# ascentai/diy-gym

Hardware: AMD Instinct MI355X
Metric: env steps/sec (whole node) (higher is better)
Workload: dtype f32; 1 GPU; ur_high_5 x 16384 envs per GPU; envs_total=16384, substeps=2, auto_reset=True, launch=hipGraph replay of 8-step segments, parallelism=independent env shards x1, no collective, envs_per_wavefront=64, lds_bytes_per_workgroup=160512, parity=vs the C oracle only; parity with pybullet itself is UNPINNED (DESIGN.md 4)

## Files before the change

### diy_gym_amd/csrc/dg_kernels.h

```cpp
#pragma once
#include "dg_device.h"
#include "../../include/diygym_scene.h"
#include "../../include/diygym_hip.h"

namespace dg {

#define DG_MAX_LINKS 64
#define DG_MAX_BODIES 192

#define DG_CONSTANT __attribute__((address_space(4)))
typedef const int32_t DG_CONSTANT* cip;
typedef const float DG_CONSTANT* cfp;

struct DevScene {
  cip BI, LI, FI, SI, PI, GI, OI, IL;
  cfp BF, LF, FF, SF, PF, OF, FL, HF;
  cip PLB;
  int split_pgs;
  int early_dyn;
  int coll_split, cont2_off;
  int coll_wave;
  cfp GD;
  cip AM;
  cip SD;
// ... 70 lines not shown
    A.M.xx = L(o + 15); A.M.xy = L(o + 16); A.M.xz = L(o + 17); A.M.yy = L(o + 18); A.M.yz = L(o + 19); A.M.zz = L(o + 20);
    return A;
  }
  DGD void LAIset(int o, const AI& A) const {
    L(o) = A.I.xx; L(o + 1) = A.I.xy; L(o + 2) = A.I.xz; L(o + 3) = A.I.yy; L(o + 4) = A.I.yz; L(o + 5) = A.I.zz;
    _Pragma("unroll") for (int k = 0; k < 9; k++) L(o + 6 + k) = A.H.m[k];
    L(o + 15) = A.M.xx; L(o + 16) = A.M.xy; L(o + 17) = A.M.xz; L(o + 18) = A.M.yy; L(o + 19) = A.M.yz; L(o + 20) = A.M.zz;
  }
  DGD void LAIadd(int o, const AI& A) const {
    L(o) += A.I.xx; L(o + 1) += A.I.xy; L(o + 2) += A.I.xz; L(o + 3) += A.I.yy; L(o + 4) += A.I.yz; L(o + 5) += A.I.zz;
    _Pragma("unroll") for (int k = 0; k < 9; k++) L(o + 6 + k) += A.H.m[k];
    L(o + 15) += A.M.xx; L(o + 16) += A.M.xy; L(o + 17) += A.M.xz; L(o + 18) += A.M.yy; L(o + 19) += A.M.yz; L(o + 20) += A.M.zz;
  }

  DGD cip bi(int b) const { return sc.BI + b * DG_BI_STRIDE; }
  DGD cfp bf(int b) const { return sc.BF + b * DG_BF_STRIDE; }
  DGD cip li(int l) const { return sc.LI + l * DG_LI_STRIDE; }
  DGD cfp lf(int l) const { return sc.LF + l * DG_LF_STRIDE; }
  DGD cip plb(int b) const { return sc.PLB + b * PLB_STRIDE; }
  DGD cip pll(int l) const { return sc.PLL + l * PLL_STRIDE; }
  DGD bool fixed(int b) const { return bi(b)[DG_BI_FLAGS] & DG_BODY_FIXED; }
  DGD bool frozen(int b) const { return bi(b)[DG_BI_FLAGS] & DG_BODY_FROZEN; }
  DGD int ext_off(int b) const { return bi(b)[DG_BI_STATE_OFF] + (fixed(b) ? DG_BS_FIXED_END : DG_BS_FLOAT_END); }
  DGD float mass_scale(int gl) const { const int o = li(gl)[DG_LI_MASS_SCALE]; return o >= 0 ? S(o) : 1.0f; }
  DGD float ang_damping(int b) const { const int o = bi(b)[DG_BI_DYN_OFF]; return o >= 0 ? S(o) : sc.HF[DG_HF_ANG_DAMPING]; }
  DGD void link_inertia(int gl, float& m, V3& c, Sym3& Ic) const {
    cfp f = lf(gl); m = f[DG_LF_MASS]; c = v3(f[DG_LF_COM], f[DG_LF_COM + 1], f[DG_LF_COM + 2]); Ic = sym6(f + DG_LF_INERTIA);
    if (li(gl)[DG_LI_MASS_SCALE] >= 0) { const float s = mass_scale(gl); m *= s; Ic.xx *= s; Ic.xy *= s; Ic.xz *= s; Ic.yy *= s; Ic.yz *= s; Ic.zz *= s; }
  }

  DGD V3 base_pos(int b) const {
    if (frozen(b)) { cfp f = bf(b) + DG_BF_INIT_POS; return v3(f[0], f[1], f[2]); }
    int o = bi(b)[DG_BI_STATE_OFF]; return v3(S(o), S(o + 1), S(o + 2));
  }
  DGD Q4 base_quat(int b) const {
    if (frozen(b)) { cfp f = bf(b) + DG_BF_INIT_QUAT; Q4 q = {f[0], f[1], f[2], f[3]}; return q; }
    int o = bi(b)[DG_BI_STATE_OFF] + DG_BS_QUAT; Q4 q = {S(o), S(o + 1), S(o + 2), S(o + 3)}; return q;
  }

  DGD void link_world(int b, int gl, M3& R, V3& p) const {
    if (gl < 0) { R = frozen(b) ? qmat(base_quat(b)) : LR(plb(b)[PLB_R0]); p = base_pos(b); }
    else { int o = pll(gl)[PLL_POSE]; R = LR(o); p = L3(o + 6); }
  }

  DGD void joint_xform(int gl, float q, M3& Rpc, V3& r) const {
    cfp f = lf(gl);
    M3 RT; _Pragma("unroll") for (int k = 0; k < 9; k++) RT.m[k] = f[DG_LF_ROT + k];
    V3 pT = v3(f[DG_LF_POS], f[DG_LF_POS + 1], f[DG_LF_POS + 2]);
    V3 ax = v3(f[DG_LF_AXIS], f[DG_LF_AXIS + 1], f[DG_LF_AXIS + 2]);
    if (li(gl)[DG_LI_TYPE] == 0) { Rpc = mul(RT, rot_axis(ax, q)); r = pT; }
    else { Rpc = RT; r = pT + mul(RT, ax * q); }
  }

  DGD void kinematics_chain(int b) const {
    constexpr int N = 6;
    cip B = bi(b); const int first = B[DG_BI_FIRST_LINK], n = B[DG_BI_N_LINKS];
    M3 R = qmat(base_quat(b)); V3 p = base_pos(b);
    LRset(plb(b)[PLB_R0], R);
    float qv[N];
#pragma unroll
    for (int j = 0; j < N; j++) qv[j] = S(li(first + min(j, n - 1))[DG_LI_STATE_OFF] + DG_LS_Q);
#pragma unroll
    for (int j = 0; j < N; j++) {
      if (j < n) {
        const int gl = first + j; M3 Rpc; V3 r; joint_xform(gl, qv[j], Rpc, r);
        const M3 Rn = mul(R, Rpc); p = p + mul(R, r);
        const int o = pll(gl)[PLL_POSE];
        LRset(o, Rn); L3set(o + 6, p);
        const V3 c0 = v3(Rn.m[0], Rn.m[3], Rn.m[6]), c1 = v3(Rn.m[1], Rn.m[4], Rn.m[7]), c2 = cross(c0, c1);
        const M3 Rb = {{c0.x, c1.x, c2.x, c0.y, c1.y, c2.y, c0.z, c1.z, c2.z}}; R = Rb;
      }
    }
  }
  DGD void kinematics(int b, int qoff = -1) const {
    cip B = bi(b);
    if (B[DG_BI_FLAGS] & DG_BODY_FROZEN) return;
    if (qoff < 0 && plb(b)[PLB_CHAIN]) { kinematics_chain(b); return; }
    int first = B[DG_BI_FIRST_LINK], n = B[DG_BI_N_LINKS];
    M3 R0 = qmat(base_quat(b)); V3 p0 = base_pos(b);
    LRset(plb(b)[PLB_R0], R0);
    constexpr int KCH = 8;
    for (int i0 = 0; i0 < n; i0 += KCH) {
      float qv[KCH];
#pragma unroll
      for (int j = 0; j < KCH; j++) { const int i = min(i0 + j, n - 1); qv[j] = qoff >= 0 ? L(qoff + i) : S(li(first + i)[DG_LI_STATE_OFF] + DG_LS_Q); }
#pragma unroll
      for (int j = 0; j < KCH; j++) {
        const int i = i0 + j; if (i >= n) break;
        int gl = first + i, par = li(gl)[DG_LI_PARENT];
        M3 Rpc; V3 r; joint_xform(gl, qv[j], Rpc, r);
        M3 Rp; V3 pp;
        if (par < 0) { Rp = R0; pp = p0; } else { int o = pll(par)[PLL_POSE]; Rp = LR(o); pp = L3(o + 6); }
        int o = pll(gl)[PLL_POSE];
        LRset(o, mul(Rp, Rpc)); L3set(o + 6, pp + mul(Rp, r));
      }
    }
  }

  DGD void frame_state(int b, int fr, bool com, V3& p, Q4& q, V3& v, V3& w, bool want_vel) const {
    V3 off; Q4 qo; int gl;
    if (fr < 0) {
      gl = -1;
      if (com) { cfp f = bf(b); off = v3(f[DG_BF_REPORT_POS], f[DG_BF_REPORT_POS + 1], f[DG_BF_REPORT_POS + 2]);
        Q4 t = {f[DG_BF_REPORT_QUAT], f[DG_BF_REPORT_QUAT + 1], f[DG_BF_REPORT_QUAT + 2], f[DG_BF_REPORT_QUAT + 3]}; qo = t; }
      else { off = v3(0, 0, 0); Q4 t = {0, 0, 0, 1}; qo = t; }
    } else {
      gl = sc.FI[fr * DG_FI_STRIDE + DG_FI_LINK];
      cfp f = sc.FF + fr * DG_FF_STRIDE + (com ? DG_FF_COM_POS : DG_FF_POS);
      off = v3(f[0], f[1], f[2]); Q4 t = {f[3], f[4], f[5], f[6]}; qo = t;
    }
    M3 R; V3 o; link_world(b, gl, R, o);
    Q4 ql = gl < 0 ? base_quat(b) : qfrom_mat(R);
    p = o + mul(R, off); q = qnormalize(qmul(ql, qo));
    if (!want_vel) return;
    V3 wl = v3(0, 0, 0), vl = v3(0, 0, 0), po = base_pos(b);
    if (!fixed(b)) { int so = bi(b)[DG_BI_STATE_OFF]; vl = v3(S(so + DG_BS_LINVEL), S(so + DG_BS_LINVEL + 1), S(so + DG_BS_LINVEL + 2));
      wl = v3(S(so + DG_BS_ANGVEL), S(so + DG_BS_ANGVEL + 1), S(so + DG_BS_ANGVEL + 2)); }
    if (gl >= 0) {
      int first = bi(b)[DG_BI_FIRST_LINK];
      unsigned long long path = 0ull; for (int k = gl; k >= 0; k = li(k)[DG_LI_PARENT]) path |= 1ull << (k - first);
      for (int k = first; k <= gl; k++) {
        if (!((path >> (k - first)) & 1ull)) continue;
        int po_off = pll(k)[PLL_POSE]; M3 Rk = LR(po_off); V3 pk = L3(po_off + 6);
        cfp f = lf(k); V3 axw = mul(Rk, v3(f[DG_LF_AXIS], f[DG_LF_AXIS + 1], f[DG_LF_AXIS + 2]));
        float qd = S(li(k)[DG_LI_STATE_OFF] + DG_LS_QD);
        vl = vl + cross(wl, pk - po);
        if (li(k)[DG_LI_TYPE] == 0) wl = wl + axw * qd; else vl = vl + axw * qd;
        po = pk;
      }
    }
    w = wl; v = vl + cross(wl, p - po);
  }

// ... 402 lines not shown
```

### diy_gym_amd/csrc/dg_solver.h

```cpp
#pragma once
#include "dg_kernels.h"
#include "dg_hull.h"

namespace dg {

enum { PS_UPDATE = 0, PS_KIN, PS_COLLIDE, PS_ABA, PS_MINV, PS_ROWS, PS_PGS, PS_INTEGRATE, PS_OUTPUT, PS_PGS_MOTOR, PS_PGS_LIMIT, PS_PGS_CONTACT, PS_COUNT,
       PS_ROW = PS_COUNT + 12  };
template <bool PROF> struct Prof;
template <> struct Prof<false> { DGD void start() {} DGD void stamp(int) {} };
template <> struct Prof<true> {
  unsigned long long last, acc[PS_COUNT];
  DGD void start() { _Pragma("unroll") for (int k = 0; k < PS_COUNT; k++) acc[k] = 0ull; last = __builtin_amdgcn_s_memtime(); }
  DGD void stamp(int id) {
    unsigned long long t = __builtin_amdgcn_s_memtime();
    _Pragma("unroll") for (int k = 0; k < PS_COUNT; k++) if (k == id) acc[k] += t - last;
    last = t;
  }
};

struct WShape { int type, body, glink; M3 R; V3 p; float prm0, prm1, prm2, mu; int poff, npts; };

template <int LANES>
DGD void shape_world(const Lane<LANES>& ln, int sh, WShape& o) {
  cip si = ln.sc.SI + sh * DG_SI_STRIDE; cfp sf = ln.sc.SF + sh * DG_SF_STRIDE;
// ... 2291 lines not shown
    }
    float U[21];
#pragma unroll
    for (int k = 0; k < 21; k++) U[k] = 0.f;
    for (int k = 0; k < n; k++) {
      float col[6];
#pragma unroll
      for (int r = 0; r < 6; r++) col[r] = ln.L(jo + r * n + k);
#pragma unroll
      for (int r = 0; r < 6; r++)
#pragma unroll
        for (int c = 0; c <= r; c++) U[r * (r + 1) / 2 + c] += col[r] * col[c];
    }
#pragma unroll
    for (int r = 0; r < 6; r++) U[r * (r + 1) / 2 + r] += lam2;
    chol6(U);
    float y[6]; chol6_solve(U, dS, y);
    float Jv[6] = {0.f, 0.f, 0.f, 0.f, 0.f, 0.f};
    for (int k = 0; k < n; k++) {
      float t = 0.f;
#pragma unroll
      for (int r = 0; r < 6; r++) t += ln.L(jo + r * n + k) * y[r];
      float v0 = 0.f;
      if (nullsp) {
        float q = ln.L(qo + k), lo = rest[n + k], hi = rest[2 * n + k], rg = rest[3 * n + k];
        v0 = g0 * (rest[k] - q);
        if (q > hi) v0 += g1 * (hi - q) / rg;
        if (q < lo) v0 += g1 * (lo - q) / rg;
#pragma unroll
        for (int r = 0; r < 6; r++) Jv[r] += ln.L(jo + r * n + k) * v0;
      }
      ln.L(vo + k) = v0; ln.L(dto + k) = t;
    }
    float mx = 0.f;
    if (nullsp) {
      float z[6]; chol6_solve(U, Jv, z);
      for (int k = 0; k < n; k++) {
        float t = 0.f;
#pragma unroll
        for (int r = 0; r < 6; r++) t += ln.L(jo + r * n + k) * z[r];
        float d = ln.L(dto + k) + ln.L(vo + k) - t; ln.L(dto + k) = d; mx = fmaxf(mx, fabsf(d));
      }
    } else {
      for (int k = 0; k < n; k++) mx = fmaxf(mx, fabsf(ln.L(dto + k)));
    }
    const float scl = mx > maxang ? maxang / mx : 1.0f;
    for (int k = 0; k < n; k++) if (live) ln.L(qo + k) += scl * ln.L(dto + k);
  }
  return iters;
}

#define DG_IK_DEV_CHAIN 256
#define DG_IK_DEV_FULL 512
template <int LANES, int N, bool FULL = false, bool NS = false, bool ORN = false>
DGD int run_ik_chain(const Lane<LANES>& ln, int op, const float* act, bool live_lane, float* qout) {
  const DevScene& sc = ln.sc; cip oi = sc.OI + op * DG_OI_STRIDE;
  const int b = oi[DG_OI_BODY], fr = oi[DG_OI_FRAME], flags = oi[DG_OI_FLAGS];
  const bool use_orn = FULL ? ORN : (flags & DG_IK_USE_ORIENTATION) != 0, nullsp = FULL ? NS : (flags & DG_IK_NULLSPACE) != 0;
  const int first = ln.bi(b)[DG_BI_FIRST_LINK], n = FULL ? N : ln.bi(b)[DG_BI_N_LINKS];
  const int eel = FULL ? N - 1 : sc.FI[fr * DG_FI_STRIDE + DG_FI_LINK] - first;
  cfp rest = sc.FL + oi[DG_OI_FLIST]; cfp ff = sc.FF + fr * DG_FF_STRIDE;
  const V3 off = v3(ff[DG_FF_COM_POS], ff[DG_FF_COM_POS + 1], ff[DG_FF_COM_POS + 2]);
  const Q4 qoff = {ff[DG_FF_COM_QUAT], ff[DG_FF_COM_QUAT + 1], ff[DG_FF_COM_QUAT + 2], ff[DG_FF_COM_QUAT + 3]};
  const M3 R0 = ln.LR(ln.plb(b)[PLB_R0]); const V3 p0 = ln.base_pos(b);
  float q[N]; V3 ow[N], aw[N];
  float cR[N][9], cP[N][3]; bool rev[N];
  M3 Qprev = {{1.f, 0.f, 0.f, 0.f, 1.f, 0.f, 0.f, 0.f, 1.f}}, Qee = Qprev;
#pragma unroll
  for (int i = 0; i < N; i++) {
    q[i] = 0.f; rev[i] = true;
#pragma unroll
    for (int k = 0; k < 9; k++) cR[i][k] = 0.f;
#pragma unroll
    for (int k = 0; k < 3; k++) cP[i][k] = 0.f;
    if (FULL || i < n) {
      cfp f = ln.lf(first + i); q[i] = ln.S(ln.li(first + i)[DG_LI_STATE_OFF] + DG_LS_Q); rev[i] = FULL || ln.li(first + i)[DG_LI_TYPE] == 0;
      M3 RT; _Pragma("unroll") for (int k = 0; k < 9; k++) RT.m[k] = pin(f[DG_LF_ROT + k]);
      const V3 pT = v3(pin(f[DG_LF_POS]), pin(f[DG_LF_POS + 1]), pin(f[DG_LF_POS + 2]));
      const V3 ax = v3(pin(f[DG_LF_AXIS]), pin(f[DG_LF_AXIS + 1]), pin(f[DG_LF_AXIS + 2]));
      V3 u, v; tangent_basis(ax, u, v);
      const M3 Qi = {{u.x, v.x, ax.x, u.y, v.y, ax.y, u.z, v.z, ax.z}};
      const M3 RTp = mul(transpose(Qprev), mul(RT, Qi)); const V3 pTp = tmul(Qprev, pT);
#pragma unroll
      for (int k = 0; k < 9; k++) cR[i][k] = RTp.m[k];
      cP[i][0] = pTp.x; cP[i][1] = pTp.y; cP[i][2] = pTp.z;
      Qprev = Qi; if (FULL ? i == N - 1 : i == eel) Qee = Qi;
    }
  }
  const V3 offp = tmul(Qee, off);
  float nRest[N], nLo[N], nHi[N], nIrg[N];
#pragma unroll
  for (int i = 0; i < N; i++) {
    nRest[i] = 0.f; nLo[i] = -3.0e38f; nHi[i] = 3.0e38f; nIrg[i] = 0.f;
    if (nullsp && (FULL || i < n)) { nRest[i] = pin(rest[i]); nLo[i] = pin(rest[n + i]); nHi[i] = pin(rest[2 * n + i]); nIrg[i] = pin(frcp(rest[3 * n + i])); }
  }
  V3 pe; M3 Re;
  auto fk = [&]() {
    M3 R = R0; V3 p = p0; M3 Rl = R0; V3 pl = p0;
#pragma unroll
    for (int i = 0; i < N; i++) {
      if (FULL || i < n) {
        M3 RT; _Pragma("unroll") for (int k = 0; k < 9; k++) RT.m[k] = cR[i][k];
        p = p + mul(R, v3(cP[i][0], cP[i][1], cP[i][2]));
        const M3 C = mul(R, RT);
        const V3 c0 = v3(C.m[0], C.m[3], C.m[6]), c1 = v3(C.m[1], C.m[4], C.m[7]), c2 = v3(C.m[2], C.m[5], C.m[8]);
        if (FULL || rev[i]) {
          const float sn = __sinf(q[i]), cs = __cosf(q[i]);
          const V3 n0 = c0 * cs + c1 * sn, n1 = c1 * cs - c0 * sn;
          const M3 Rn = {{n0.x, n1.x, c2.x, n0.y, n1.y, c2.y, n0.z, n1.z, c2.z}}; R = Rn;
        } else { R = C; p = p + c2 * q[i]; }
        ow[i] = p; aw[i] = c2;
        if (FULL ? i == N - 1 : i == eel) { Rl = R; pl = p; }
      }
    }
    pe = pl + mul(Rl, offp); Re = Rl;
  };
  fk();
  const V3 tp = pe + v3(act[0], act[1], act[2]);
  M3 Tm = {{1.f, 0.f, 0.f, 0.f, 1.f, 0.f, 0.f, 0.f, 1.f}};
  if (use_orn) {
    const Q4 qe0 = qnormalize(qmul(qfrom_mat(mul(Re, transpose(Qee))), qoff));
    const Q4 tq = qmul(qe0, qfrom_euler(act[3], act[4], act[5]));
    Tm = mul(mul(qmat(tq), transpose(qmat(qoff))), Qee);
  }
  const float lam2 = nullsp ? sc.HF[DG_HF_IK_LAMBDA_SQ] : sc.HF[DG_HF_IK_JOINT_DAMPING], maxang = sc.HF[DG_HF_IK_MAX_ANGLE], g0 = sc.HF[DG_HF_IK_NULL_REST_GAIN], g1 = sc.HF[DG_HF_IK_NULL_LIMIT_GAIN];
  const float resid = sc.HF[DG_HF_IK_RESIDUAL];
  bool live = live_lane; int iters = 0;
  for (int it = 0; it < sc.ik_iters; it++) {
    if (it > 0) fk();
    const V3 ep = tp - pe;
    if (it > 0 && norm(ep) < resid) live = false;
    if (!__any(live)) break;
    iters += live ? 1 : 0;
    float dS[6] = {ep.x, ep.y, ep.z, 0.f, 0.f, 0.f};
    if (use_orn) {
      const float* T = Tm.m; const float* R = Re.m;
      const float tr = T[0] * R[0] + T[1] * R[1] + T[2] * R[2] + T[3] * R[3] + T[4] * R[4] + T[5] * R[5] + T[6] * R[6] + T[7] * R[7] + T[8] * R[8];
      const float m21 = T[3] * R[0] + T[4] * R[1] + T[5] * R[2], m12 = T[0] * R[3] + T[1] * R[4] + T[2] * R[5];
      const float m31 = T[6] * R[0] + T[7] * R[1] + T[8] * R[2], m13 = T[0] * R[6] + T[1] * R[7] + T[2] * R[8];
      const float m32 = T[6] * R[3] + T[7] * R[4] + T[8] * R[5], m23 = T[3] * R[6] + T[4] * R[7] + T[5] * R[8];
      const float sx = 0.5f * (m32 - m23), sy = 0.5f * (m13 - m31), sz = 0.5f * (m21 - m12);
      const float sn = fsqrt(sx * sx + sy * sy + sz * sz), an = atan2f(sn, 0.5f * (tr - 1.0f)), k = sn > 1e-12f ? fdiv(an, sn) : 1.0f;
      dS[3] = sx * k; dS[4] = sy * k; dS[5] = sz * k;
    }
    float U[21], Jv[6] = {0.f, 0.f, 0.f, 0.f, 0.f, 0.f}, v0[N], cols[N][6];
#pragma unroll
    for (int k = 0; k < 21; k++) U[k] = 0.f;
    auto column = [&](int i, float* col) {
      const V3 jl = (FULL || rev[i]) ? cross(aw[i], pe - ow[i]) : aw[i]; const V3 ja = ((FULL || rev[i]) && use_orn) ? aw[i] : v3(0.f, 0.f, 0.f);
      col[0] = jl.x; col[1] = jl.y; col[2] = jl.z; col[3] = ja.x; col[4] = ja.y; col[5] = ja.z;
    };
#pragma unroll
    for (int i = 0; i < N; i++) {
      v0[i] = 0.f;
      if (FULL || i < n) {
        if (nullsp) {
          v0[i] = g0 * (nRest[i] - q[i]);
          if (q[i] > nHi[i]) v0[i] += g1 * (nHi[i] - q[i]) * nIrg[i];
          if (q[i] < nLo[i]) v0[i] += g1 * (nLo[i] - q[i]) * nIrg[i];
        }
        if (FULL || i <= eel) {
          float* col = cols[i]; column(i, col);
#pragma unroll
          for (int r = 0; r < 6; r++) {
            Jv[r] += col[r] * v0[i];
#pragma unroll
            for (int c = 0; c <= r; c++) U[r * (r + 1) / 2 + c] += col[r] * col[c];
          }
        }
      }
    }
#pragma unroll
    for (int r = 0; r < 6; r++) U[r * (r + 1) / 2 + r] += lam2;
    chol6(U);
    float rhs[6], y[6];
#pragma unroll
    for (int r = 0; r < 6; r++) rhs[r] = dS[r] - Jv[r];
    chol6_solve(U, rhs, y);
    float dth[N], mx = 0.f;
#pragma unroll
    for (int i = 0; i < N; i++) {
      dth[i] = 0.f;
      if (FULL || i < n) {
        float t = 0.f;
        if (FULL || i <= eel) {
#pragma unroll
          for (int r = 0; r < 6; r++) t += cols[i][r] * y[r];
        }
        dth[i] = t + v0[i]; mx = fmaxf(mx, fabsf(dth[i]));
      }
    }
    const float scl = mx > maxang ? fdiv(maxang, mx) : 1.0f;
#pragma unroll
    for (int i = 0; i < N; i++) if ((FULL || i < n) && live) q[i] += scl * dth[i];
  }
#pragma unroll
  for (int i = 0; i < N; i++) qout[i] = q[i];
  return iters;
}

typedef float v2f __attribute__((ext_vector_type(2)));
DGD v2f sp2(float s) { v2f r = {s, s}; return r; }
DGD v2f fma2(v2f a, v2f b, v2f c) { return __builtin_elementwise_fma(a, b, c); }
struct P3 { v2f xy; float z; };
DGD P3 p3(V3 v) { P3 r; r.xy.x = v.x; r.xy.y = v.y; r.z = v.z; return r; }
DGD P3 colmul_acc(const P3& c0, const P3& c1, const P3& c2, float x, float y, float z, const P3& acc) {
  P3 r; r.xy = fma2(c2.xy, sp2(z), fma2(c1.xy, sp2(y), fma2(c0.xy, sp2(x), acc.xy))); r.z = fmaf(c2.z, z, fmaf(c1.z, y, fmaf(c0.z, x, acc.z))); return r;
}
DGD P3 colmul(const P3& c0, const P3& c1, const P3& c2, float x, float y, float z) {
  P3 r; r.xy = fma2(c2.xy, sp2(z), fma2(c1.xy, sp2(y), c0.xy * sp2(x))); r.z = fmaf(c2.z, z, fmaf(c1.z, y, c0.z * x)); return r;
}
template <int LANES, bool ORN>
DGD int run_ik_chain_pk(const Lane<LANES>& ln, int op, const float* act, bool live_lane, float* qout) {
  constexpr int N = 6;
  const DevScene& sc = ln.sc; cip oi = sc.OI + op * DG_OI_STRIDE;
  const int b = oi[DG_OI_BODY], fr = oi[DG_OI_FRAME];
  const int first = ln.bi(b)[DG_BI_FIRST_LINK];
  cfp rest = sc.FL + oi[DG_OI_FLIST]; cfp ff = sc.FF + fr * DG_FF_STRIDE;
  const V3 off = v3(ff[DG_FF_COM_POS], ff[DG_FF_COM_POS + 1], ff[DG_FF_COM_POS + 2]);
  const Q4 qoff = {ff[DG_FF_COM_QUAT], ff[DG_FF_COM_QUAT + 1], ff[DG_FF_COM_QUAT + 2], ff[DG_FF_COM_QUAT + 3]};
  const M3 R0 = ln.LR(ln.plb(b)[PLB_R0]); const V3 p0 = ln.base_pos(b);
  float q[N];
  float cR[N][9], cP[N][3];
  M3 Qprev = {{1.f, 0.f, 0.f, 0.f, 1.f, 0.f, 0.f, 0.f, 1.f}}, Qee = Qprev;
#pragma unroll
  for (int i = 0; i < N; i++) {
    cfp f = ln.lf(first + i); q[i] = ln.S(ln.li(first + i)[DG_LI_STATE_OFF] + DG_LS_Q);
    M3 RT; _Pragma("unroll") for (int k = 0; k < 9; k++) RT.m[k] = pin(f[DG_LF_ROT + k]);
    const V3 pT = v3(pin(f[DG_LF_POS]), pin(f[DG_LF_POS + 1]), pin(f[DG_LF_POS + 2]));
    const V3 ax = v3(pin(f[DG_LF_AXIS]), pin(f[DG_LF_AXIS + 1]), pin(f[DG_LF_AXIS + 2]));
    V3 u, v; tangent_basis(ax, u, v);
    const M3 Qi = {{u.x, v.x, ax.x, u.y, v.y, ax.y, u.z, v.z, ax.z}};
    const M3 RTp = mul(transpose(Qprev), mul(RT, Qi)); const V3 pTp = tmul(Qprev, pT);
#pragma unroll
    for (int k = 0; k < 9; k++) cR[i][k] = RTp.m[k];
    cP[i][0] = pTp.x; cP[i][1] = pTp.y; cP[i][2] = pTp.z;
    Qprev = Qi; if (i == N - 1) Qee = Qi;
  }
  const V3 offp = tmul(Qee, off);
  float nRest[N], nLo[N], nHi[N], nIrg[N];
#pragma unroll
  for (int i = 0; i < N; i++) { nRest[i] = pin(rest[i]); nLo[i] = pin(rest[N + i]); nHi[i] = pin(rest[2 * N + i]); nIrg[i] = pin(frcp(rest[3 * N + i])); }
  const P3 b0 = p3(v3(R0.m[0], R0.m[3], R0.m[6])), b1 = p3(v3(R0.m[1], R0.m[4], R0.m[7])), b2 = p3(v3(R0.m[2], R0.m[5], R0.m[8])), bp = p3(p0);
  P3 ow[N], aw[N], pe, e0, e1, e2;
  auto fk = [&]() {
    P3 c0 = b0, c1 = b1, c2 = b2, p = bp;
#pragma unroll
    for (int i = 0; i < N; i++) {
      const float* T = cR[i];
      p = colmul_acc(c0, c1, c2, cP[i][0], cP[i][1], cP[i][2], p);
      const P3 C0 = colmul(c0, c1, c2, T[0], T[3], T[6]), C1 = colmul(c0, c1, c2, T[1], T[4], T[7]), C2 = colmul(c0, c1, c2, T[2], T[5], T[8]);
      const float sn = __sinf(q[i]), cs = __cosf(q[i]);
      P3 n0, n1;
      n0.xy = fma2(C1.xy, sp2(sn), C0.xy * sp2(cs)); n0.z = fmaf(C1.z, sn, C0.z * cs);
      n1.xy = fma2(C0.xy, sp2(-sn), C1.xy * sp2(cs)); n1.z = fmaf(C0.z, -sn, C1.z * cs);
      c0 = n0; c1 = n1; c2 = C2; ow[i] = p; aw[i] = C2;
    }
    pe = colmul_acc(c0, c1, c2, offp.x, offp.y, offp.z, p); e0 = c0; e1 = c1; e2 = c2;
  };
  fk();
  const V3 pe0 = v3(pe.xy.x, pe.xy.y, pe.z);
  const V3 tp = pe0 + v3(act[0], act[1], act[2]);
  M3 Tm = {{1.f, 0.f, 0.f, 0.f, 1.f, 0.f, 0.f, 0.f, 1.f}};
  if (ORN) {
    const M3 Re = {{e0.xy.x, e1.xy.x, e2.xy.x, e0.xy.y, e1.xy.y, e2.xy.y, e0.z, e1.z, e2.z}};
    const Q4 qe0 = qnormalize(qmul(qfrom_mat(mul(Re, transpose(Qee))), qoff));
    const Q4 tq = qmul(qe0, qfrom_euler(act[3], act[4], act[5]));
    Tm = mul(mul(qmat(tq), transpose(qmat(qoff))), Qee);
  }
  const float lam2 = sc.HF[DG_HF_IK_LAMBDA_SQ], maxang = sc.HF[DG_HF_IK_MAX_ANGLE], g0 = sc.HF[DG_HF_IK_NULL_REST_GAIN], g1 = sc.HF[DG_HF_IK_NULL_LIMIT_GAIN];
  const float resid = sc.HF[DG_HF_IK_RESIDUAL];
  bool live = live_lane; int iters = 0;
  for (int it = 0; it < sc.ik_iters; it++) {
    if (it > 0) fk();
    const v2f epxy = v2f{tp.x, tp.y} - pe.xy; const float epz = tp.z - pe.z;
    if (it > 0 && fsqrt(epxy.x * epxy.x + epxy.y * epxy.y + epz * epz) < resid) live = false;
    if (!__any(live)) break;
    iters += live ? 1 : 0;
    v2f dA = epxy, dB = {0.f, 0.f}, dC = {epz, 0.f};
    if (ORN) {
      const P3 M0 = colmul(e0, e1, e2, Tm.m[0], Tm.m[1], Tm.m[2]), M1 = colmul(e0, e1, e2, Tm.m[3], Tm.m[4], Tm.m[5]), M2 = colmul(e0, e1, e2, Tm.m[6], Tm.m[7], Tm.m[8]);
      const float tr = M0.xy.x + M1.xy.y + M2.z;
      const float sx = 0.5f * (M2.xy.y - M1.z), sy = 0.5f * (M0.z - M2.xy.x), sz = 0.5f * (M1.xy.x - M0.xy.y);
      const float sn = fsqrt(sx * sx + sy * sy + sz * sz), an = atan2f(sn, 0.5f * (tr - 1.0f)), k = sn > 1e-12f ? fdiv(an, sn) : 1.0f;
      dB = v2f{sx * k, sy * k}; dC.y = sz * k;
    }
    float U00 = 0.f, U22 = 0.f, U44 = 0.f; v2f U1 = {0.f, 0.f}, U2a = U1, U3a = U1, U3b = U1, U4a = U1, U4b = U1, U5a = U1, U5b = U1, U5c = U1;
    v2f JvA = U1, JvB = U1, JvC = U1, cA[N], cB[N], cC[N]; float v0[N];
#pragma unroll
    for (int i = 0; i < N; i++) {
      float v = g0 * (nRest[i] - q[i]);
      if (q[i] > nHi[i]) v += g1 * (nHi[i] - q[i]) * nIrg[i];
      if (q[i] < nLo[i]) v += g1 * (nLo[i] - q[i]) * nIrg[i];
      v0[i] = v;
      const v2f dxy = pe.xy - ow[i].xy; const float dz = pe.z - ow[i].z; const P3& a = aw[i];
      const v2f pa = {a.xy.y, -a.xy.x}, pd = {dxy.y, -dxy.x};
      const v2f A = fma2(pa, sp2(dz), -(pd * sp2(a.z)));
      const float lz = a.xy.x * dxy.y - a.xy.y * dxy.x;
      const v2f B = a.xy, C = {lz, a.z};
      cA[i] = A; cB[i] = B; cC[i] = C;
      JvA = fma2(A, sp2(v), JvA); JvB = fma2(B, sp2(v), JvB); JvC = fma2(C, sp2(v), JvC);
      U00 = fmaf(A.x, A.x, U00); U1 = fma2(A, sp2(A.y), U1);
      U2a = fma2(A, sp2(B.x), U2a); U22 = fmaf(B.x, B.x, U22);
      U3a = fma2(A, sp2(B.y), U3a); U3b = fma2(B, sp2(B.y), U3b);
      U4a = fma2(A, sp2(C.x), U4a); U4b = fma2(B, sp2(C.x), U4b); U44 = fmaf(C.x, C.x, U44);
      U5a = fma2(A, sp2(C.y), U5a); U5b = fma2(B, sp2(C.y), U5b); U5c = fma2(C, sp2(C.y), U5c);
    }
    float U[21] = {U00 + lam2, U1.x, U1.y + lam2, U2a.x, U2a.y, U22 + lam2, U3a.x, U3a.y, U3b.x, U3b.y + lam2,
                   U4a.x, U4a.y, U4b.x, U4b.y, U44 + lam2, U5a.x, U5a.y, U5b.x, U5b.y, U5c.x, U5c.y + lam2};
    chol6(U);
    const float rhs[6] = {dA.x - JvA.x, dA.y - JvA.y, dB.x - JvB.x, dB.y - JvB.y, dC.x - JvC.x, dC.y - JvC.y};
    float y[6]; chol6_solve(U, rhs, y);
// ... 28 lines not shown
DGD M3 qmat_x(Q4 q) {
#pragma clang fp contract(off)
  const float n = q.x * q.x + q.y * q.y + q.z * q.z + q.w * q.w, s = n > 0.f ? 2.0f * __frcp_rn(n) : 0.f;
  const float xs = q.x * s, ys = q.y * s, zs = q.z * s;
  const float wx = q.w * xs, wy = q.w * ys, wz = q.w * zs, xx = q.x * xs, xy = q.x * ys, xz = q.x * zs, yy = q.y * ys, yz = q.y * zs, zz = q.z * zs;
  M3 R = {{1.f - (yy + zz), xy - wz, xz + wy, xy + wz, 1.f - (xx + zz), yz - wx, xz - wy, yz + wx, 1.f - (xx + yy)}};
  return R;
}
DGD float spool_up(float w, float a, float k) {
#pragma clang fp contract(off)
  const float d = a - w; const float p = d * k; return w + p;
}
DGD float mul_sep(float a, float b) {
#pragma clang fp contract(off)
  const float p = a * b; return p;
}
DGD V3 mulx(const M3& R, V3 v) {
#pragma clang fp contract(off)
  return v3(R.m[0] * v.x + R.m[1] * v.y + R.m[2] * v.z, R.m[3] * v.x + R.m[4] * v.y + R.m[5] * v.z, R.m[6] * v.x + R.m[7] * v.y + R.m[8] * v.z);
}
template <int LANES>
DGD void apply_frame_wrench(const Lane<LANES>& ln, int b, int fr, V3 f, V3 pos, V3 t, bool link_frame) {
#pragma clang fp contract(off)
  const DevScene& sc = ln.sc;
  const int gl = fr < 0 ? -1 : sc.FI[fr * DG_FI_STRIDE + DG_FI_LINK];
  V3 F = f, T = t, P = pos;
  if (link_frame) {
    V3 fp; M3 R;
    if (gl < 0) {
      const Q4 qb = ln.base_quat(b); const V3 pb = ln.base_pos(b);
      cfp ff = fr >= 0 ? sc.FF + fr * DG_FF_STRIDE + DG_FF_COM_POS : ln.bf(b) + DG_BF_REPORT_POS;
      const V3 off = v3(ff[0], ff[1], ff[2]); const Q4 qo = {ff[3], ff[4], ff[5], ff[6]};
      const V3 ro = mulx(qmat_x(qb), off); fp = v3(pb.x + ro.x, pb.y + ro.y, pb.z + ro.z); R = qmat_x(qnormalize_x(qmul_x(qb, qo)));
    } else { V3 fv, fw; Q4 fq; ln.frame_state(b, fr, true, fp, fq, fv, fw, false); R = qmat_x(fq); }
    F = mulx(R, f); T = mulx(R, t);
    const V3 rp = mulx(R, pos); P = v3(fp.x + rp.x, fp.y + rp.y, fp.z + rp.z);
  }
  if (!ln.fixed(b)) {
    const V3 bp = ln.base_pos(b), r = v3(P.x - bp.x, P.y - bp.y, P.z - bp.z);
    const V3 tq = v3((r.y * F.z - r.z * F.y) + T.x, (r.z * F.x - r.x * F.z) + T.y, (r.x * F.y - r.y * F.x) + T.z); const int eo = ln.ext_off(b);
    ln.Sset(eo, ln.S(eo) + F.x); ln.Sset(eo + 1, ln.S(eo + 1) + F.y); ln.Sset(eo + 2, ln.S(eo + 2) + F.z);
    ln.Sset(eo + 3, ln.S(eo + 3) + tq.x); ln.Sset(eo + 4, ln.S(eo + 4) + tq.y); ln.Sset(eo + 5, ln.S(eo + 5) + tq.z);
  }
  for (int k = gl; k >= 0; k = ln.li(k)[DG_LI_PARENT]) {
    const int po = ln.pll(k)[PLL_POSE], lo = ln.li(k)[DG_LI_STATE_OFF]; cfp lf = ln.lf(k);
    const M3 Rk = ln.LR(po); const V3 pk = ln.L3(po + 6), a = v3(lf[DG_LF_AXIS], lf[DG_LF_AXIS + 1], lf[DG_LF_AXIS + 2]);
    const V3 axw = v3(Rk.m[0] * a.x + Rk.m[1] * a.y + Rk.m[2] * a.z, Rk.m[3] * a.x + Rk.m[4] * a.y + Rk.m[5] * a.z, Rk.m[6] * a.x + Rk.m[7] * a.y + Rk.m[8] * a.z);
    const V3 r = v3(P.x - pk.x, P.y - pk.y, P.z - pk.z), m = v3((r.y * F.z - r.z * F.y) + T.x, (r.z * F.x - r.x * F.z) + T.y, (r.x * F.y - r.y * F.x) + T.z);
    const float tau = ln.li(k)[DG_LI_TYPE] == 0 ? axw.x * m.x + axw.y * m.y + axw.z * m.z : axw.x * F.x + axw.y * F.y + axw.z * F.z;
    ln.Sset(lo + DG_LS_TORQUE, ln.S(lo + DG_LS_TORQUE) + tau);
  }
}

template <int LANES>
DGD void run_update_ops(const Lane<LANES>& ln, const float* act_row, uint64_t mask, int only_body = -1, int skip_body = -1, int32_t* diag = nullptr) {
  const DevScene& sc = ln.sc; int ik_ord = -1;
  for (int op = 0; op < sc.nops; op++) {
    cip oi = sc.OI + op * DG_OI_STRIDE; cfp of = sc.OF + op * DG_OF_STRIDE; const int code = oi[DG_OI_CODE];
    if (code == DG_OP_IK_CONTROL) ik_ord++;
    if (code < DG_OP_JOINT_CONTROL || code > DG_OP_ADMITTANCE) continue;
    if ((only_body >= 0 && oi[DG_OI_BODY] != only_body) || oi[DG_OI_BODY] == skip_body) continue;
    if (!((mask >> oi[DG_OI_SLOT]) & 1ull)) continue;
    const float* a = act_row + oi[DG_OI_IO_OFF]; cip il = sc.IL + oi[DG_OI_ILIST]; const int n = oi[DG_OI_N];
    if (code == DG_OP_JOINT_CONTROL) {
      const int mode = oi[DG_OI_FLAGS];
      for (int k = 0; k < n; k++) {
        const int lo = ln.li(il[k])[DG_LI_STATE_OFF];
        if (mode == DG_JC_POSITION) { ln.Sset(lo + DG_LS_TARGET_POS, a[k]); ln.Sset(lo + DG_LS_TARGET_VEL, 0.f); }
        else if (mode == DG_JC_VELOCITY) { ln.Sset(lo + DG_LS_TARGET_VEL, a[k]); ln.Sset(lo + DG_LS_TARGET_POS, 0.f); }
        else ln.Sset(lo + DG_LS_TORQUE, a[k]);
      }
    } else if (code == DG_OP_IK_CONTROL) {
      const int b = oi[DG_OI_BODY];
      float av[6] = {a[0], a[1], a[2], 0.f, 0.f, 0.f};
      if (oi[DG_OI_FLAGS] & DG_IK_USE_ORIENTATION) { av[3] = a[3]; av[4] = a[4]; av[5] = a[5]; }
      if (oi[DG_OI_FLAGS] & DG_IK_DEV_CHAIN) {
        float qs[6]; int ik_it;
        const int fl = oi[DG_OI_FLAGS];
        if ((fl & DG_IK_DEV_FULL) && (fl & DG_IK_NULLSPACE) && (fl & DG_IK_USE_ORIENTATION)) ik_it = run_ik_chain_pk<LANES, true>(ln, op, av, ln.valid, qs);
        else if ((fl & DG_IK_DEV_FULL) && (fl & DG_IK_NULLSPACE)) ik_it = run_ik_chain_pk<LANES, false>(ln, op, av, ln.valid, qs);
        else ik_it = run_ik_chain<LANES, 6>(ln, op, av, ln.valid, qs);
        if (diag && ln.valid && ik_ord < DG_DIAG_N_IK) diag[(size_t)DG_DIAG_STRIDE * ln.env + DG_DIAG_IK_ITERS + ik_ord] = ik_it;
        const int first = ln.bi(b)[DG_BI_FIRST_LINK];
        for (int k = 0; k < n; k++) {
          const int lo = ln.li(il[k])[DG_LI_STATE_OFF], j = il[k] - first; float v = qs[0];
#pragma unroll
          for (int c = 1; c < 6; c++) v = (j == c) ? qs[c] : v;
          ln.Sset(lo + DG_LS_TARGET_POS, v); ln.Sset(lo + DG_LS_TARGET_VEL, 0.f);
        }
        continue;
      }
      { const int ik_it = run_ik(ln, op, av, ln.valid);
        if (diag && ln.valid && ik_ord < DG_DIAG_N_IK) diag[(size_t)DG_DIAG_STRIDE * ln.env + DG_DIAG_IK_ITERS + ik_ord] = ik_it; }
      for (int k = 0; k < n; k++) {
        const int lo = ln.li(il[k])[DG_LI_STATE_OFF];
        ln.Sset(lo + DG_LS_TARGET_POS, ln.L(sc.tr_off + (il[k] - ln.bi(b)[DG_BI_FIRST_LINK]))); ln.Sset(lo + DG_LS_TARGET_VEL, 0.f);
      }
      ln.kinematics(b);
    } else if (code == DG_OP_ADMITTANCE) {
      const int b = oi[DG_OI_BODY], first = ln.bi(b)[DG_BI_FIRST_LINK], nl = ln.bi(b)[DG_BI_N_LINKS];
      V3 fp, fv, fw; Q4 fq; ln.frame_state(b, oi[DG_OI_FRAME], true, fp, fq, fv, fw, false);
      const V3 pw = fp + mul(qmat(fq), v3(of[0], of[1], of[2]));
      const int eel = sc.FI[oi[DG_OI_FRAME] * DG_FI_STRIDE + DG_FI_LINK];
      const V3 F = v3(a[0], a[1], a[2]), T = v3(a[3], a[4], a[5]), g = v3(sc.gx, sc.gy, sc.gz); cfp tgt = sc.FL + oi[DG_OI_FLIST];
      for (int k = 0; k < n; k++) {
        const int gl = il[k], lo = ln.li(gl)[DG_LI_STATE_OFF], po = ln.pll(gl)[PLL_POSE]; cfp f = ln.lf(gl);
        const M3 Rj = ln.LR(po); const V3 oj = ln.L3(po + 6), axw = mul(Rj, v3(f[DG_LF_AXIS], f[DG_LF_AXIS + 1], f[DG_LF_AXIS + 2]));
        const bool rev = ln.li(gl)[DG_LI_TYPE] == 0;
        bool anc = false; for (int i = eel; i >= 0; i = ln.li(i)[DG_LI_PARENT]) if (i == gl) anc = true;
        float tau = 0.f;
        if (anc) tau += rev ? dot(F, cross(axw, pw - oj)) + dot(T, axw) : dot(F, axw);
        for (int i = first; i < first + nl; i++) {
          bool sub = false; for (int q = i; q >= 0; q = ln.li(q)[DG_LI_PARENT]) if (q == gl) sub = true;
          if (!sub) continue;
          cfp fi2 = ln.lf(i); const int pi2 = ln.pll(i)[PLL_POSE];
          const V3 cw = ln.L3(pi2 + 6) + mul(ln.LR(pi2), v3(fi2[DG_LF_COM], fi2[DG_LF_COM + 1], fi2[DG_LF_COM + 2])); const V3 w8 = g * (fi2[DG_LF_MASS] * ln.mass_scale(i));
          tau -= rev ? dot(w8, cross(axw, cw - oj)) : dot(w8, axw);
        }
        tau += of[3] * (tgt[k] - ln.S(lo + DG_LS_Q)) - of[4] * ln.S(lo + DG_LS_QD);
        ln.Sset(lo + DG_LS_TORQUE, ln.S(lo + DG_LS_TORQUE) + tau);
      }
    } else if (code == DG_OP_EXTERNAL_FORCE) {
      const int b = oi[DG_OI_BODY]; if (ln.fixed(b)) continue;
      apply_frame_wrench(ln, b, -1, v3(a[0], a[1], a[2]), v3(of[0], of[1], of[2]), v3(0.f, 0.f, 0.f), false);
    } else if (code == DG_OP_PROPELLOR) {
      const int b = oi[DG_OI_BODY], so = sc.addon_off + oi[DG_OI_STATE_OFF];
      const float w = spool_up(ln.S(so), a[0], of[2]); ln.Sset(so, w);
      if (ln.fixed(b)) continue;
      apply_frame_wrench(ln, b, oi[DG_OI_FRAME], v3(0.f, 0.f, mul_sep(of[0], w)), v3(0.f, 0.f, 0.f), v3(0.f, 0.f, mul_sep(of[1], w)), true);
    }
  }
}

template <int LANES>
// ... 234 lines not shown
```

### diy_gym_amd/csrc/dg_step_par_body.inc

```
  constexpr int reset_mode = DG_PAR_RESET;
  extern __shared__ float smem[];
  const int wave = threadIdx.x >> 6, lane = threadIdx.x & 63;
  const int env = blockIdx.x * 64 + lane; const bool exists = env < sc.num_envs; const int e = exists ? env : sc.num_envs - 1;
  const bool doit = exists && (!reset_mode || reset_mask == nullptr || reset_mask[e] != 0);
  if (reset_mode && !__any(doit)) return;
  const bool valid = reset_mode ? doit : exists;
  const float* act_row = actions ? actions + (size_t)e * sc.act_dim : nullptr;
  const unsigned long long t_start = PROF ? __builtin_amdgcn_s_memtime() : 0ull; (void)t_start;
  if (wave == 3) {
    Lane<64> ln(sc, mt, smem + lane, state + e, e, valid);
    if (reset_mode) __syncthreads();
    DG_WAVE_STAMP(0); __syncthreads();
    if (sc.early_dyn) {
      early_dynamics(ln, 1);
      if (sc.coll_split) collide<64, 64>(ln, sc.npairs / 2, 0x7fffffff, sc.cont2_off);
    }
    DG_WAVE_STAMP(1); __syncthreads();
    for (int k = 0; k < sc.substeps; k++) {
      __syncthreads();
      if (sc.coll_split && !(sc.early_dyn && k == 0)) collide<64, 64>(ln, sc.npairs / 2, 0x7fffffff, sc.cont2_off);
      __syncthreads();
      if (!substep_contact_free(ln) && split_decide_follow(ln, 0u, false)) __syncthreads();
      __syncthreads();
    }
    DG_WAVE_STAMP(2); __syncthreads();
    run_output_ops(ln, nullptr, (valid && rew) ? rew + (size_t)e * sc.rew_dim : nullptr, (valid && term) ? term + (size_t)e * sc.term_dim : nullptr,
                   (valid && rew_sum) ? rew_sum + e : nullptr, (valid && term_flag) ? term_flag + e : nullptr, OUT_REW_TERM);
    DG_WAVE_STAMP(3);
    return;
  }
  if (wave == 2) {
    Lane<64> ln(sc, mt, smem + lane, state + e, e, valid);
    if (reset_mode) __syncthreads();
    DG_WAVE_STAMP(0); __syncthreads();
    if (sc.early_dyn) {
      collide<64, 64>(ln, 0, sc.coll_split ? sc.npairs / 2 : 0x7fffffff);
      early_dynamics(ln, 0);
    }
    DG_WAVE_STAMP(1); __syncthreads();
    for (int k = 0; k < sc.substeps; k++) {
      __syncthreads();
      if (sc.coll_wave && !(sc.early_dyn && k == 0)) collide<64, 64>(ln, 0, sc.coll_split ? sc.npairs / 2 : 0x7fffffff);
      __syncthreads();
      if (!substep_contact_free(ln) && split_decide_follow(ln, false, false)) __syncthreads();
      __syncthreads();
    }
    DG_WAVE_STAMP(2); __syncthreads();
    run_output_ops(ln, (valid && obs) ? obs + (size_t)e * sc.obs_dim : nullptr, nullptr, nullptr, nullptr, nullptr, OUT_OBS_REST);
    DG_WAVE_STAMP(3);
    return;
  }
  if (wave == 1) {
    Lane<64> ln(sc, mt, smem + lane, state + e, e, valid);
    if (reset_mode) __syncthreads();
    ln.kinematics(sc.helper_body);
    DG_WAVE_STAMP(0); __syncthreads();
    if (act_row) run_update_ops(ln, act_row, mask, sc.helper_body, -1, diag);
    DG_WAVE_STAMP(1); __syncthreads();
    for (int k = 0; k < sc.substeps; k++) helper_substep(ln, sc.early_dyn && k == 0, k == sc.substeps - 1);
    ln.kinematics(sc.helper_body);
    DG_WAVE_STAMP(2); __syncthreads();
    run_output_ops(ln, (valid && obs) ? obs + (size_t)e * sc.obs_dim : nullptr, nullptr, nullptr, nullptr, nullptr, OUT_JOINT_OF, sc.helper_body);
    DG_WAVE_STAMP(3);
    return;
  }
  Lane<64> ln(sc, mt, smem + lane, state + e, e, valid);
  Prof<PROF> prof; prof.start();
  if (reset_mode) { if (doit) { ln.Sset(DG_ST_STEP, 0.0f); run_reset_ops(ln); } __syncthreads(); }
  for (int b = 0; b < sc.nba; b++) if (b != sc.helper_body) ln.kinematics(b);
  __syncthreads();
  prof.stamp(PS_KIN);
  if (act_row) run_update_ops(ln, act_row, mask, -1, sc.helper_body, diag);
  if (!reset_mode) ln.Sset(DG_ST_STEP, ln.S(DG_ST_STEP) + 1.0f);
  __syncthreads();
  prof.stamp(PS_UPDATE);
  sim_step<64, PROF, true>(ln, diag, prof);
  for (int b = 0; b < sc.nba; b++) if (b != sc.helper_body) ln.kinematics(b);
  __syncthreads();
  prof.stamp(PS_KIN);
  run_output_ops(ln, (valid && obs) ? obs + (size_t)e * sc.obs_dim : nullptr, nullptr, nullptr, nullptr, nullptr, OUT_JOINT_NOT_OF, sc.helper_body);
  prof.stamp(PS_OUTPUT);
  if constexpr (PROF) { if (lane == 0) for (int k = 0; k < PS_COUNT; k++) cycles[(size_t)blockIdx.x * PS_ROW + k] = prof.acc[k]; }
```

Before: 182.3 million env-steps/s.

## Hand off pre-step link kinematics to idle waves and overlap with IK start

When early dynamics and split collision are enabled, the full link-pose kinematics for the helper body and first regular body moves to waves 3 and 2, which are otherwise idle before the first barrier. The IK-owning waves only write the base rotation to LDS and then begin IK. A Handover functor places the first barrier inside the IK routine, just before its forward-kinematics pass, so per-op constant loads and setup overlap with the pose computation on other waves. This shortens the serial kinematics-then-update critical path, at the cost of extra template plumbing and barrier placement that depends on IK being reached.

Measured after the change: 188.8 million env-steps/s (median of 6 runs). 3.6% higher.

```diff
diff --git a/diy_gym_amd/csrc/dg_kernels.h b/diy_gym_amd/csrc/dg_kernels.h
--- a/diy_gym_amd/csrc/dg_kernels.h
+++ b/diy_gym_amd/csrc/dg_kernels.h
@@ -146,11 +146,12 @@
     else { Rpc = RT; r = pT + mul(RT, ax * q); }
   }
 
-  DGD void kinematics_chain(int b) const {
+  DGD void base_rot_to_lds(int b) const { if (!frozen(b)) LRset(plb(b)[PLB_R0], qmat(base_quat(b))); }
+  DGD void kinematics_chain(int b, bool base_rot = true) const {
     constexpr int N = 6;
     cip B = bi(b); const int first = B[DG_BI_FIRST_LINK], n = B[DG_BI_N_LINKS];
     M3 R = qmat(base_quat(b)); V3 p = base_pos(b);
-    LRset(plb(b)[PLB_R0], R);
+    if (base_rot) LRset(plb(b)[PLB_R0], R);
     float qv[N];
 #pragma unroll
     for (int j = 0; j < N; j++) qv[j] = S(li(first + min(j, n - 1))[DG_LI_STATE_OFF] + DG_LS_Q);
@@ -166,13 +167,13 @@
       }
     }
   }
-  DGD void kinematics(int b, int qoff = -1) const {
+  DGD void kinematics(int b, int qoff = -1, bool base_rot = true) const {
     cip B = bi(b);
     if (B[DG_BI_FLAGS] & DG_BODY_FROZEN) return;
-    if (qoff < 0 && plb(b)[PLB_CHAIN]) { kinematics_chain(b); return; }
+    if (qoff < 0 && plb(b)[PLB_CHAIN]) { kinematics_chain(b, base_rot); return; }
     int first = B[DG_BI_FIRST_LINK], n = B[DG_BI_N_LINKS];
     M3 R0 = qmat(base_quat(b)); V3 p0 = base_pos(b);
-    LRset(plb(b)[PLB_R0], R0);
+    if (base_rot) LRset(plb(b)[PLB_R0], R0);
     constexpr int KCH = 8;
     for (int i0 = 0; i0 < n; i0 += KCH) {
       float qv[KCH];
diff --git a/diy_gym_amd/csrc/dg_solver.h b/diy_gym_amd/csrc/dg_solver.h
--- a/diy_gym_amd/csrc/dg_solver.h
+++ b/diy_gym_amd/csrc/dg_solver.h
@@ -2367,8 +2367,15 @@
 
 #define DG_IK_DEV_CHAIN 256
 #define DG_IK_DEV_FULL 512
-template <int LANES, int N, bool FULL = false, bool NS = false, bool ORN = false>
-DGD int run_ik_chain(const Lane<LANES>& ln, int op, const float* act, bool live_lane, float* qout) {
+struct NoHandover { DGD void operator()() const {} };
+template <class F>
+struct Handover {
+  F f; bool done;
+  DGD Handover(F fn, bool d) : f(fn), done(d) {}
+  DGD void operator()() { if (!done) { done = true; f(); } }
+};
+template <int LANES, int N, bool FULL = false, bool NS = false, bool ORN = false, class HO = NoHandover>
+DGD int run_ik_chain(const Lane<LANES>& ln, int op, const float* act, bool live_lane, float* qout, HO&& ho = HO()) {
   const DevScene& sc = ln.sc; cip oi = sc.OI + op * DG_OI_STRIDE;
   const int b = oi[DG_OI_BODY], fr = oi[DG_OI_FRAME], flags = oi[DG_OI_FLAGS];
   const bool use_orn = FULL ? ORN : (flags & DG_IK_USE_ORIENTATION) != 0, nullsp = FULL ? NS : (flags & DG_IK_NULLSPACE) != 0;
@@ -2430,6 +2437,7 @@
     }
     pe = pl + mul(Rl, offp); Re = Rl;
   };
+  ho();
   fk();
   const V3 tp = pe + v3(act[0], act[1], act[2]);
   M3 Tm = {{1.f, 0.f, 0.f, 0.f, 1.f, 0.f, 0.f, 0.f, 1.f}};
@@ -2525,8 +2533,8 @@
 DGD P3 colmul(const P3& c0, const P3& c1, const P3& c2, float x, float y, float z) {
   P3 r; r.xy = fma2(c2.xy, sp2(z), fma2(c1.xy, sp2(y), c0.xy * sp2(x))); r.z = fmaf(c2.z, z, fmaf(c1.z, y, c0.z * x)); return r;
 }
-template <int LANES, bool ORN>
-DGD int run_ik_chain_pk(const Lane<LANES>& ln, int op, const float* act, bool live_lane, float* qout) {
+template <int LANES, bool ORN, class HO = NoHandover>
+DGD int run_ik_chain_pk(const Lane<LANES>& ln, int op, const float* act, bool live_lane, float* qout, HO&& ho = HO()) {
   constexpr int N = 6;
   const DevScene& sc = ln.sc; cip oi = sc.OI + op * DG_OI_STRIDE;
   const int b = oi[DG_OI_BODY], fr = oi[DG_OI_FRAME];
@@ -2573,6 +2581,7 @@
     }
     pe = colmul_acc(c0, c1, c2, offp.x, offp.y, offp.z, p); e0 = c0; e1 = c1; e2 = c2;
   };
+  ho();
   fk();
   const V3 pe0 = v3(pe.xy.x, pe.xy.y, pe.z);
   const V3 tp = pe0 + v3(act[0], act[1], act[2]);
@@ -2707,8 +2716,8 @@
   }
 }
 
-template <int LANES>
-DGD void run_update_ops(const Lane<LANES>& ln, const float* act_row, uint64_t mask, int only_body = -1, int skip_body = -1, int32_t* diag = nullptr) {
+template <int LANES, class HO = NoHandover>
+DGD void run_update_ops(const Lane<LANES>& ln, const float* act_row, uint64_t mask, int only_body = -1, int skip_body = -1, int32_t* diag = nullptr, HO&& ho = HO()) {
   const DevScene& sc = ln.sc; int ik_ord = -1;
   for (int op = 0; op < sc.nops; op++) {
     cip oi = sc.OI + op * DG_OI_STRIDE; cfp of = sc.OF + op * DG_OF_STRIDE; const int code = oi[DG_OI_CODE];
@@ -2732,9 +2741,9 @@
       if (oi[DG_OI_FLAGS] & DG_IK_DEV_CHAIN) {
         float qs[6]; int ik_it;
         const int fl = oi[DG_OI_FLAGS];
-        if ((fl & DG_IK_DEV_FULL) && (fl & DG_IK_NULLSPACE) && (fl & DG_IK_USE_ORIENTATION)) ik_it = run_ik_chain_pk<LANES, true>(ln, op, av, ln.valid, qs);
-        else if ((fl & DG_IK_DEV_FULL) && (fl & DG_IK_NULLSPACE)) ik_it = run_ik_chain_pk<LANES, false>(ln, op, av, ln.valid, qs);
-        else ik_it = run_ik_chain<LANES, 6>(ln, op, av, ln.valid, qs);
+        if ((fl & DG_IK_DEV_FULL) && (fl & DG_IK_NULLSPACE) && (fl & DG_IK_USE_ORIENTATION)) ik_it = run_ik_chain_pk<LANES, true>(ln, op, av, ln.valid, qs, ho);
+        else if ((fl & DG_IK_DEV_FULL) && (fl & DG_IK_NULLSPACE)) ik_it = run_ik_chain_pk<LANES, false>(ln, op, av, ln.valid, qs, ho);
+        else ik_it = run_ik_chain<LANES, 6>(ln, op, av, ln.valid, qs, ho);
         if (diag && ln.valid && ik_ord < DG_DIAG_N_IK) diag[(size_t)DG_DIAG_STRIDE * ln.env + DG_DIAG_IK_ITERS + ik_ord] = ik_it;
         const int first = ln.bi(b)[DG_BI_FIRST_LINK];
         for (int k = 0; k < n; k++) {
diff --git a/diy_gym_amd/csrc/dg_step_par_body.inc b/diy_gym_amd/csrc/dg_step_par_body.inc
--- a/diy_gym_amd/csrc/dg_step_par_body.inc
+++ b/diy_gym_amd/csrc/dg_step_par_body.inc
@@ -7,9 +7,11 @@
   const bool valid = reset_mode ? doit : exists;
   const float* act_row = actions ? actions + (size_t)e * sc.act_dim : nullptr;
   const unsigned long long t_start = PROF ? __builtin_amdgcn_s_memtime() : 0ull; (void)t_start;
+  const bool pose_ho = sc.early_dyn && sc.coll_split;
   if (wave == 3) {
     Lane<64> ln(sc, mt, smem + lane, state + e, e, valid);
     if (reset_mode) __syncthreads();
+    if (pose_ho) ln.kinematics(sc.helper_body, -1, false);
     DG_WAVE_STAMP(0); __syncthreads();
     if (sc.early_dyn) {
       early_dynamics(ln, 1);
@@ -32,6 +34,7 @@
   if (wave == 2) {
     Lane<64> ln(sc, mt, smem + lane, state + e, e, valid);
     if (reset_mode) __syncthreads();
+    if (pose_ho) ln.kinematics(sc.reg_body[0], -1, false);
     DG_WAVE_STAMP(0); __syncthreads();
     if (sc.early_dyn) {
       collide<64, 64>(ln, 0, sc.coll_split ? sc.npairs / 2 : 0x7fffffff);
@@ -53,9 +56,10 @@
   if (wave == 1) {
     Lane<64> ln(sc, mt, smem + lane, state + e, e, valid);
     if (reset_mode) __syncthreads();
-    ln.kinematics(sc.helper_body);
-    DG_WAVE_STAMP(0); __syncthreads();
-    if (act_row) run_update_ops(ln, act_row, mask, sc.helper_body, -1, diag);
+    Handover b0([&]() { DG_WAVE_STAMP(0); __syncthreads(); }, false);
+    if (pose_ho) ln.base_rot_to_lds(sc.helper_body); else { ln.kinematics(sc.helper_body); b0(); }
+    if (act_row) run_update_ops(ln, act_row, mask, sc.helper_body, -1, diag, b0);
+    b0();
     DG_WAVE_STAMP(1); __syncthreads();
     for (int k = 0; k < sc.substeps; k++) helper_substep(ln, sc.early_dyn && k == 0, k == sc.substeps - 1);
     ln.kinematics(sc.helper_body);
@@ -67,10 +71,12 @@
   Lane<64> ln(sc, mt, smem + lane, state + e, e, valid);
   Prof<PROF> prof; prof.start();
   if (reset_mode) { if (doit) { ln.Sset(DG_ST_STEP, 0.0f); run_reset_ops(ln); } __syncthreads(); }
-  for (int b = 0; b < sc.nba; b++) if (b != sc.helper_body) ln.kinematics(b);
-  __syncthreads();
+  Handover b0([&]() { __syncthreads(); }, false);
+  for (int b = 0; b < sc.nba; b++) if (b != sc.helper_body) { if (pose_ho && b == sc.reg_body[0]) ln.base_rot_to_lds(b); else ln.kinematics(b); }
+  if (!pose_ho) b0();
   prof.stamp(PS_KIN);
-  if (act_row) run_update_ops(ln, act_row, mask, -1, sc.helper_body, diag);
+  if (act_row) run_update_ops(ln, act_row, mask, -1, sc.helper_body, diag, b0);
+  b0();
   if (!reset_mode) ln.Sset(DG_ST_STEP, ln.S(DG_ST_STEP) + 1.0f);
   __syncthreads();
   prof.stamp(PS_UPDATE);
```
